# princeton-computational-imaging/Neural-Volume-Super-Resolution

Measured on AMD Instinct MI355X. Metric: rendered rays/sec (64+128 samples) at 800x800 Lego-like view, higher is better.
Workload: dtype f32 as 2 f16 limbs (3 MFMA products, f32 acc); 1 GPU; Blender-'lego'-like 800x800 view, 64 coarse + 128 fine samples, tri-plane decoder (3x800^2x48 + 32^2x48 planes, 4+4x128 MLP), 1 view per GPU per step; partition=view

## Files before the change

### neural-volume-super-resolution_amd/csrc/pair_core.h

```cpp
#pragma once
#include <type_traits>
#include <utility>

#ifndef R3_DMA_AUX
#define R3_DMA_AUX 0
#endif
#ifndef R3_ABLATE
#define R3_ABLATE 0
#endif
#include "limb_core.h"
#include "side_work.h"

#ifndef R3_GATHER_NT
#define R3_GATHER_NT 0
#endif
#ifndef R3_STAMP
#define R3_STAMP 0
#endif
#if R3_STAMP == 4
#define R3_MARK(i)
#define R3_MARKB(i)
#define R3_RESET
#define R3_MARKH(i) { __builtin_amdgcn_sched_barrier(0); const unsigned long long t_ = __builtin_amdgcn_s_memtime(); stamp[i] += (float)(t_ - tprev); tprev = t_; __builtin_amdgcn_sched_barrier(0); }
#define R3_RESETH { tprev = __builtin_amdgcn_s_memtime(); }
#elif R3_STAMP == 3
#define R3_MARKH(i)
#define R3_RESETH
#define R3_MARK(i)
#define R3_MARKB(i) { __builtin_amdgcn_sched_barrier(0); const unsigned long long t_ = __builtin_amdgcn_s_memtime(); stamp[i] += (float)(t_ - tprev); tprev = t_; __builtin_amdgcn_sched_barrier(0); }
#define R3_RESET { tprev = __builtin_amdgcn_s_memtime(); }
#elif R3_STAMP
#define R3_MARKB(i)
#define R3_RESET
#define R3_MARKH(i)
#define R3_RESETH
#define R3_MARK(i) { __builtin_amdgcn_sched_barrier(0); const unsigned long long t_ = __builtin_amdgcn_s_memtime(); stamp[i] += (float)(t_ - tprev); tprev = t_; __builtin_amdgcn_sched_barrier(0); }
#else
#define R3_MARK(i)
#define R3_MARKB(i)
#define R3_RESET
#define R3_MARKH(i)
#define R3_RESETH
#endif
#ifndef R3_RELU_PK
#define R3_RELU_PK 0
#endif
#ifndef R3_BLEND_PK
#define R3_BLEND_PK 0
#endif
#ifndef R3_NO_VIEW_HOIST
#define R3_NO_VIEW_HOIST 1
#endif

namespace nvsr {

template <int LIMBS>
struct Lds3 {
    static constexpr int SLOT = 4 * kb_words(LIMBS);
    static constexpr int SMALL = 2 * SLOT;
    static constexpr int RAYS = SMALL + SMALL_FLOATS;
    static constexpr int RAY_FLOATS = LIMBS == 2 ? 8 : 20;
    static constexpr int TAP_FLOATS = LIMBS == 2 ? 8 : 0;
    static constexpr int VTAPS = RAYS + RAYS2 * RAY_FLOATS;
    static constexpr int FAR = LIMBS == 2 ? VTAPS + RAYS2 * TAP_FLOATS : -1;
    static constexpr int RES = VTAPS + RAYS2 * TAP_FLOATS + (LIMBS == 2 ? RAYS2 : 0);
    static constexpr int RES_KB = LIMBS == 2 ? 9 : 0;
    static constexpr int PTS_WORDS = 8 * RAYS2;
    static constexpr int PTS = LIMBS == 2 ? VTAPS : RES + RES_KB * kb_words(LIMBS);
    static_assert(LIMBS != 2 || RAYS2 * TAP_FLOATS >= PTS_WORDS, "the points' region fits the taps'");
    static constexpr int TOTAL = RES + RES_KB * kb_words(LIMBS) + (LIMBS == 2 ? 0 : PTS_WORDS);
};
static_assert(Lds3<3>::TOTAL * 4 <= 160 * 1024 && Lds3<2>::TOTAL * 4 <= 160 * 1024, "LDS budget");

struct Tile3 {
    f32x16 acc[4];
    f32x16 act[4];
    float D[HALF_C], F[HALF_C];
    float V[HALF_C];
    float T, cr, cg, cb, dep, ac, zc, zn;
    float raw[4];
};

struct RawTaps4 { f32x4 r[4][HALF_C / 4]; };
constexpr int GATHER_STEPS = 12 + HALF_C;
__device__ __forceinline__ void gather4_load(int k, const GatherJob& job, int h, RawTaps4& rt) {
    const int tap = k / 3, i0 = 2 * (k % 3);
#if R3_ABLATE & 1
    rt.r[tap][i0] = f32x4{job.t.nw, job.t.ne, job.t.sw, job.t.se};
    rt.r[tap][i0 + 1] = f32x4{job.t.se, job.t.ne, job.t.sw, job.t.nw};
    return;
#endif
    const int off = tap == 0 ? job.t.o00 : tap == 1 ? job.t.o01 : tap == 2 ? job.t.o10 : job.t.o11;
    const f32x4* p = reinterpret_cast<const f32x4*>(job.plane + off + HALF_C * h);
    rt.r[tap][i0] = p[i0];
    rt.r[tap][i0 + 1] = p[i0 + 1];
}
__device__ __forceinline__ void gather4_blend(int c, const GatherJob& job, const RawTaps4& rt, float (&F)[HALF_C]) {
    const int i = c >> 2, j = c & 3;
    F[c] = fmaf(rt.r[3][i][j], job.t.se, fmaf(rt.r[2][i][j], job.t.sw, fmaf(rt.r[1][i][j], job.t.ne, rt.r[0][i][j] * job.t.nw)));
}

template <int NS, bool LOADS, bool BLENDS, bool PK = false>
__device__ __forceinline__ void gather_roll(int slot, const GatherJob& jl, float (&Fl)[HALF_C], const GatherJob& jb, float (&Fb)[HALF_C], int h,
                                            RawTaps4& rt) {
    spread<72, 0, NS>(slot, [&](int v) {
        if (LOADS && v % 3 == 0) {
            const int tap = (v / 3) / 6, piece = (v / 3) % 6;
#if R3_ABLATE & 1
            rt.r[tap][piece] = f32x4{jl.t.nw, jl.t.ne, jl.t.sw, jl.t.se};
#else
            int off = tap == 0 ? jl.t.o00 : tap == 1 ? jl.t.o01 : tap == 2 ? jl.t.o10 : jl.t.o11;
#if R3_ABLATE & 2
            off = __builtin_amdgcn_readfirstlane(off);
#endif
#if R3_ABLATE & 4
            off = off & 0xffff;
            off -= off % 48;
#endif
#if R3_GATHER_NT
            rt.r[tap][piece] = __builtin_nontemporal_load(reinterpret_cast<const f32x4*>(jl.plane + off + HALF_C * h) + piece);
#else
            rt.r[tap][piece] = reinterpret_cast<const f32x4*>(jl.plane + off + HALF_C * h)[piece];
#endif
#endif
        }
        const int w = v / 18, u = v % 18;
        if constexpr (PK) {
            if (u % 3 != 2) {
                const int c = 2 * ((u / 3) * 2 + u % 3);
                if (LOADS && w == 3) {
                    f32x2_t m = f32x2_t{rt.r[0][c >> 2][c & 3], rt.r[0][c >> 2][(c & 3) + 1]} * f32x2_t{jl.t.nw, jl.t.nw};
// ... 163 lines not shown
```

### neural-volume-super-resolution_amd/csrc/render3.hip

```cpp
#include "pair_core.h"

#include "colour_order.h"
#include "occupancy.h"
#include "nvsr_internal.h"

namespace nvsr {

template <int LZ>
__device__ __forceinline__ void render_pass3_body(const SceneDev& sc, const float* __restrict__ packed, long N, int S,
                                                  const float* __restrict__ rays, const float* __restrict__ z, int lindisp,
                                                  const float* __restrict__ noise, int white,
                                                  float* __restrict__ rgb, float* __restrict__ disp,
                                                  float* __restrict__ acc, float* __restrict__ weights,
                                                  float* __restrict__ depth, float* __restrict__ raw_out, unsigned* __restrict__ flag,
                                                  float* __restrict__ live_z = nullptr, float* __restrict__ live_w = nullptr,
                                                  int* __restrict__ live_n = nullptr, const int* __restrict__ group_slot = nullptr,
                                                  const int* __restrict__ pts = nullptr, const int* __restrict__ pt_steps = nullptr, float* views = nullptr,
                                                  const int* __restrict__ kept = nullptr, const int* __restrict__ kept_n = nullptr) {
    constexpr int LIMBS = LZ & 7;
    constexpr bool ZCOMP = (LZ & 8) != 0;
    constexpr int PHASE = (LZ >> 4) & 7;
    constexpr bool FUSED = PHASE == 0, KEPT = PHASE == 4, DENSITY = PHASE == 1 || KEPT, POINTS = PHASE == 3, COLOUR = PHASE == 2 || POINTS;
    using L = Lds3<LIMBS>;
    constexpr int NP = limb_products(LIMBS);
// ... 149 lines not shown
        n2 = norm_coord(__fadd_rn(c0[2], __fmul_rn(c1[1], zc)), sc.lo[2], sc.range[2]);
    };
    auto scale_taps = [](Taps& t) NVSR_INL {
        if constexpr (LIMBS == 2) { t.nw *= F16_X_SCALE; t.ne *= F16_X_SCALE; t.sw *= F16_X_SCALE; t.se *= F16_X_SCALE; }
    };
    auto view_job = [&](const float* rtp) NVSR_INL {
        const f32x4 c2 = reinterpret_cast<const f32x4*>(rtp)[0], c3 = reinterpret_cast<const f32x4*>(rtp)[1];
        GatherJob j;
        j.plane = sc.plane[3];
        j.t.o00 = __float_as_int(c2[0]); j.t.o01 = __float_as_int(c2[1]); j.t.o10 = __float_as_int(c2[2]); j.t.o11 = __float_as_int(c2[3]);
        j.t.nw = c3[0]; j.t.ne = c3[1]; j.t.sw = c3[2]; j.t.se = c3[3];
        scale_taps(j.t);
        return j;
    };

    __syncthreads();
    if constexpr (!DENSITY) {
#pragma unroll
        for (int k2 = 0; k2 < 2; ++k2) {
            Tile3& t = k2 ? Y : X;
            const GatherJob vj = view_job(k2 ? rtY : rtX);
#pragma unroll
            for (int k = 0; k < 12; ++k) gather4_load(k, vj, lane0 >> 5, rt);
#pragma unroll
            for (int c = 0; c < HALF_C; ++c) gather4_blend(c, vj, rt, t.V);
        }
        if constexpr (POINTS) {
#pragma unroll
            for (int k2 = 0; k2 < 2; ++k2) {
                const Tile3& t = k2 ? Y : X;
                f32x4* vp = reinterpret_cast<f32x4*>(views + ((long)blk * RAYS2 + (k2 ? ownY : ownX)) * POINT_VIEW_FLOATS + HALF_C * (lane0 >> 5));
#pragma unroll
                for (int i = 0; i < HALF_C / 4; ++i) vp[i] = f32x4{t.V[4 * i], t.V[4 * i + 1], t.V[4 * i + 2], t.V[4 * i + 3]};
            }
            __syncthreads();
            if (lane0 < 32) {
#pragma unroll
                for (int c = 0; c < 3; ++c) pt_sums[ownX * 3 + c] = pt_sums[ownY * 3 + c] = 0.0f;
                pt_ray[ownX] = (int)(rayX - pt_block); pt_ray[ownY] = (int)(rayY - pt_block);
            }
            __syncthreads();
            const int eX0 = trip > 0 ? peX[0] : POINT_NONE, eY0 = trip > 0 ? peX[32] : POINT_NONE;
            eX1 = trip > 1 ? peX[RAYS2] : POINT_NONE; eY1 = trip > 1 ? peX[RAYS2 + 32] : POINT_NONE;
            point_of(eX0, ownX, slotX, liveX, X.zc, wX);
            point_of(eY0, ownY, slotY, liveY, Y.zc, wY);
            load_view(slotX, X.V); load_view(slotY, Y.V);
        }
    } else {
#pragma unroll
        for (int k2 = 0; k2 < 2; ++k2) {
            Tile3& t = k2 ? Y : X;
            float n0, n1, n2;
            point_norm(k2 ? rcY : rcX, t.zc, n0, n1, n2);
#pragma unroll
            for (int p = 0; p < 3; ++p) {
                GatherJob pj;
                pj.plane = sc.plane[p]; pj.t = pos_taps2(sc, p, n0, n1, n2); scale_taps(pj.t);
#pragma unroll
                for (int k = 0; k < 12; ++k) gather4_load(k, pj, lane0 >> 5, rt);
#pragma unroll
                for (int c = 0; c < HALF_C; ++c) gather4_blend(c, pj, rt, t.F);
#pragma unroll
                for (int c = 0; c < HALF_C; ++c) {
                    t.D[c] = p == 0 ? t.F[c] : p == 1 ? __fadd_rn(t.D[c], t.F[c]) : div3(__fadd_rn(t.D[c], t.F[c]));
                    asm volatile("" : "+v"(t.D[c]));
                }
                __builtin_amdgcn_sched_barrier(0);
            }
        }
    }
    Limbs<LIMBS> cur, fa;
    f32x2_t nsc = {-F16_ACC_UNSCALE, -F16_ACC_UNSCALE};
    asm volatile("" : "+s"(nsc));
#if R3_STAMP
    float stamp[8] = {0, 0, 0, 0, 0, 0, 0, 0};
    unsigned long long tprev = __builtin_amdgcn_s_memtime();
#endif
    constexpr bool RESIDENT = L::RES_KB > 0 && !DENSITY;
    constexpr int KB_FIRST = DENSITY ? KB_DEN0 : RESIDENT ? KB_RGB0 + 9 : KB_RGB0;
    unsigned* const res = lds + L::RES;
    if constexpr (RESIDENT) ring3_load_resident<LIMBS, L::RES_KB>(rs, res, KB_RGB0);
    unsigned* cw = const_cast<unsigned*>(ring3_issue<LIMBS, 3>(rs, KB_FIRST));
    const int steps = COLOUR || KEPT ? trip : S;
    for (int s = 0; s < steps; ++s) {
        asm volatile("" : "+v"(rs.voff), "+v"(rs.lane));
#if R3_NO_VIEW_HOIST
        if constexpr (!POINTS) {
#pragma unroll
        for (int c = 0; c < HALF_C; ++c) asm volatile("" : "+v"(X.V[c]), "+v"(Y.V[c]));
        }
#endif
        if constexpr (POINTS) { rcX = ldsf + L::RAYS + slotX * RAY3_FLOATS; rcY = ldsf + L::RAYS + slotY * RAY3_FLOATS; }
        const int lane = rs.lane, h = lane >> 5;
        const bool last = (s + 1 == S);
        if constexpr (!COLOUR && !KEPT) {
            X.zn = depth_of(zX, rcX, last ? s : s + 1);
            Y.zn = depth_of(zY, rcY, last ? s : s + 1);
        }
        const float nzX = !COLOUR && noise ? noise[rayX * S + s] : 0.0f;
        const float nzY = !COLOUR && noise ? noise[rayY * S + s] : 0.0f;
        float xn0, xn1, xn2, yn0, yn1, yn2;
        if constexpr (!KEPT) {
            point_norm(rcX, DENSITY ? X.zn : X.zc, xn0, xn1, xn2);
            point_norm(rcY, DENSITY ? Y.zn : Y.zc, yn0, yn1, yn2);
        }
        BiasPend4 bp;
        bp.slot = bounce_slot(ldsf + L::VTAPS + rs.wave * 64 * L::TAP_FLOATS + lane * 4);
        HeadPend<3> hp3;
        HeadPend<1> hp1;
        SplitPend tp;

        auto feat = [](const float (&f)[HALF_C]) NVSR_INL { return [&f](int kb, int i) NVSR_INL { return f[8 * kb + i]; }; };
        auto hid = [](const f32x16 (&a)[4], int kb0) NVSR_INL { return [&a, kb0](int kb, int i) NVSR_INL { const int k = kb0 + kb; return a[k >> 1][8 * (k & 1) + i]; }; };
        auto split_feat = [&](const float (&f)[HALF_C]) NVSR_INL { split_all<LIMBS>([&f](int i) NVSR_INL { return f[i]; }, cur); };
        auto tail_of = [&](const f32x16 (&a)[4], int kb) NVSR_INL {
            return [&a, kb, &tp](int slice, Limbs<LIMBS>& nxt) NVSR_INL { split_slice<LIMBS>(slice, [&a, kb](int i) NVSR_INL { return a[kb >> 1][8 * (kb & 1) + i]; }, nxt, tp); };
        };
        auto none = [](int) NVSR_INL {};

        GatherJob ja, jb;
        R3_MARK(0)
        ring3_sync<(ZCOMP || COLOUR || KEPT) ? 0 : 2>();
        int eX2 = POINT_NONE, eY2 = POINT_NONE;
        if constexpr (POINTS) {
            if (s + 2 < steps) { eX2 = peX[(s + 2) * RAYS2]; eY2 = peX[(s + 2) * RAYS2 + 32]; }
            point_of(eX1, ownX, slotXn, liveXn, X.zn, wXn);
            point_of(eY1, ownY, slotYn, liveYn, Y.zn, wYn);
        } else if constexpr (COLOUR) {
            X.zn = live_depth(lzX, rcX, nX, s + 1); Y.zn = live_depth(lzY, rcY, nY, s + 1);
            wXn = live_weight(lwX, nX, s + 1); wYn = live_weight(lwY, nY, s + 1);
        } else if constexpr (KEPT) {
            X.zn = depth_of(z_row(rayX), rcX, idxXn); Y.zn = depth_of(z_row(rayY), rcY, idxYn);
            point_norm(rcX, X.zn, xn0, xn1, xn2);
            point_norm(rcY, Y.zn, yn0, yn1, yn2);
        }
        unsigned* nw = (RESIDENT || DENSITY) ? nullptr : ring3_take(rs);
        float hx[3] = {0.0f, 0.0f, 0.0f};
        if constexpr (!DENSITY) {
        const unsigned* const w_view = RESIDENT ? res : cw;
        R3_MARK(1)
        R3_RESET
#define NVSR_ROLL(TL, JL, TB, JB, LOADS, BLENDS) [&](int slot) NVSR_INL { gather_roll<NSF, LOADS, BLENDS, LIMBS == 2 && R3_BLEND_PK>(slot, JL, TL.F, JB, TB.F, h, rt); }
#define NVSR_ROLL_DMA(TL, JL, TB, JB, LOADS, BLENDS, NKB, KB0) \
        [&](int slot) NVSR_INL { gather_roll<NSF, LOADS, BLENDS, LIMBS == 2 && R3_BLEND_PK>(slot, JL, TL.F, JB, TB.F, h, rt); dma_side<LIMBS, NKB>(slot, rs, nw, KB0); }
        ja.plane = sc.plane[0]; ja.t = pos_taps2(sc, 0, xn0, xn1, xn2); scale_taps(ja.t);
        split_feat(X.V);
        if constexpr (RESIDENT) limb_block<LIMBS, 3, true, true>(w_view, lane, X.acc, cur, fa, feat(X.V), NVSR_ROLL(X, ja, Y, jb, true, false), NoTail{});
        else limb_block<LIMBS, 3, true, true>(cw, lane, X.acc, cur, fa, feat(X.V), NVSR_ROLL_DMA(X, ja, Y, jb, true, false, 3, KB_RGB0 + 3), NoTail{});
        R3_MARKB(0)
        if constexpr (POINTS) load_view(slotXn, X.V);
        jb.plane = sc.plane[0]; jb.t = pos_taps2(sc, 0, yn0, yn1, yn2); scale_taps(jb.t);
        split_feat(Y.V);
        limb_block<LIMBS, 3, true, false>(w_view, lane, Y.acc, cur, fa, feat(Y.V), NVSR_ROLL(Y, jb, X, ja, true, true), NoTail{});
        R3_MARKB(1)
        if constexpr (POINTS) load_view(slotYn, Y.V);
        const unsigned* w_p0 = res + 3 * kb_words(LIMBS);
        if constexpr (!RESIDENT) {
            cw = nw;
            ring3_sync<YOUNGER_THAN_CHUNK>();
            nw = ring3_take(rs);
            w_p0 = cw;
        }
#pragma unroll
        for (int c = 0; c < HALF_C; ++c) X.D[c] = X.F[c];
        ja.plane = sc.plane[1]; ja.t = pos_taps2(sc, 1, xn0, xn1, xn2); scale_taps(ja.t);
        split_feat(X.F);
        if constexpr (RESIDENT) limb_block<LIMBS, 3, false, true>(w_p0, lane, X.acc, cur, fa, feat(X.F), NVSR_ROLL(X, ja, Y, jb, true, true), NoTail{});
        else limb_block<LIMBS, 3, false, true>(cw, lane, X.acc, cur, fa, feat(X.F), NVSR_ROLL_DMA(X, ja, Y, jb, true, true, 3, KB_RGB0 + 6), NoTail{});
        R3_MARKB(2)
#pragma unroll
        for (int c = 0; c < HALF_C; ++c) Y.D[c] = Y.F[c];
        jb.plane = sc.plane[1]; jb.t = pos_taps2(sc, 1, yn0, yn1, yn2); scale_taps(jb.t);
        split_feat(Y.F);
        limb_block<LIMBS, 3, false, false>(w_p0, lane, Y.acc, cur, fa, feat(Y.F), NVSR_ROLL(Y, jb, X, ja, true, true), NoTail{});
        R3_MARKB(3)
        const unsigned* w_p1 = res + 6 * kb_words(LIMBS);
        if constexpr (!RESIDENT) {
            cw = nw;
            ring3_sync<YOUNGER_THAN_CHUNK>();
            nw = ring3_take(rs);
            w_p1 = cw;
        }
#pragma unroll
        for (int c = 0; c < HALF_C; ++c) X.D[c] = __fadd_rn(X.D[c], X.F[c]);
        ja.plane = sc.plane[2]; ja.t = pos_taps2(sc, 2, xn0, xn1, xn2); scale_taps(ja.t);
        split_feat(X.F);
        if constexpr (RESIDENT) limb_block<LIMBS, 3, false, true>(w_p1, lane, X.acc, cur, fa, feat(X.F), NVSR_ROLL(X, ja, Y, jb, true, true), NoTail{});
        else limb_block<LIMBS, 3, false, true>(cw, lane, X.acc, cur, fa, feat(X.F), NVSR_ROLL_DMA(X, ja, Y, jb, true, true, 3, KB_RGB0 + 9), NoTail{});
        R3_MARKB(4)
#pragma unroll
        for (int c = 0; c < HALF_C; ++c) Y.D[c] = __fadd_rn(Y.D[c], Y.F[c]);
        jb.plane = sc.plane[2]; jb.t = pos_taps2(sc, 2, yn0, yn1, yn2); scale_taps(jb.t);
        split_feat(Y.F);
        limb_block<LIMBS, 3, false, false>(w_p1, lane, Y.acc, cur, fa, feat(Y.F), NVSR_ROLL(Y, jb, X, ja, true, true), NoTail{});
        R3_MARKB(5)
        if constexpr (!RESIDENT) {
            cw = nw;
            ring3_sync<YOUNGER_THAN_CHUNK>();
        }
        nw = ring3_take(rs);
#pragma unroll
        for (int c = 0; c < HALF_C; ++c) X.D[c] = div3(__fadd_rn(X.D[c], X.F[c]));
        split_feat(X.F);
        limb_block<LIMBS, 3, false, true>(cw, lane, X.acc, cur, fa, feat(X.F), NVSR_ROLL_DMA(X, ja, Y, jb, false, true, 4, KB_RGB1), NoTail{});
        R3_MARKB(6)
// ... 4 lines not shown
                                           [&](int slot) NVSR_INL { spread<RELU_STEPS, 0, NSF>(slot, [&](int k) NVSR_INL { relu_bias_step<LIMBS>(k, small + S_BIAS + 4 * HID, h, X.acc, X.act, bp, nsc); }); },
                                           tail_of(X.act, 0));
        R3_MARKB(7)
        cw = nw;
        R3_MARK(2)
        }

        auto relu_side = [&](Tile3& t, int bias_vec) NVSR_INL {
            return [&, bias_vec](int slot) NVSR_INL { spread<RELU_STEPS, 0, NSH>(slot, [&](int k) NVSR_INL { relu_bias_step<LIMBS>(k, small + S_BIAS + bias_vec * HID, h, t.acc, t.act, bp, nsc); }); };
        };
#define NVSR_HIDDEN_LAYER_(SYNC, XA_SIDE, VPREV, VTHIS, KB_NEXT_A, NKB_A, KB_NEXT_B, NKB_B, X_B_SIDE)                                \
        R3_RESETH                                                                                                                   \
        SYNC;                                                                                                                       \
        R3_MARKH(0)                                                                                                                 \
        nw = ring3_take(rs);                                                                                                        \
        R3_MARKH(1)                                                                                                                 \
        limb_block<LIMBS, 4, true, true>(cw, lane, X.acc, cur, fa, hid(X.act, 0),                                                   \
                                         [&](int slot) NVSR_INL { (XA_SIDE)(slot); dma_side<LIMBS, NKB_A>(slot, rs, nw, KB_NEXT_A); }, tail_of(Y.act, 0)); \
        R3_MARKH(2)                                                                                                                 \
        limb_block<LIMBS, 4, true, false>(cw, lane, Y.acc, cur, fa, hid(Y.act, 0), none, tail_of(X.act, 4));                        \
        R3_MARKH(3)                                                                                                                 \
        cw = nw;                                                                                                                    \
        ring3_sync<0>();                                                                                                               \
        nw = ring3_take(rs);                                                                                                        \
        R3_MARKH(4)                                                                                                                 \
        limb_block<LIMBS, 4, false, true>(cw, lane, X.acc, cur, fa, hid(X.act, 4),                                                  \
                                          [&](int slot) NVSR_INL { dma_side<LIMBS, NKB_B>(slot, rs, nw, KB_NEXT_B); }, tail_of(Y.act, 4));   \
        R3_MARKH(5)                                                                                                                 \
        X_B_SIDE;                                                                                                                   \
        R3_MARKH(6)                                                                                                                 \
        cw = nw;

#define NVSR_HIDDEN_LAYER(VPREV, ...) NVSR_HIDDEN_LAYER_(ring3_sync<0>(), relu_side(Y, VPREV), VPREV, __VA_ARGS__)
#define NVSR_YB_PLAIN(VTHIS) (limb_block<LIMBS, 4, false, false>(cw, lane, Y.acc, cur, fa, hid(Y.act, 4), relu_side(X, VTHIS), tail_of(X.act, 0)))
        if constexpr (!DENSITY) {
        NVSR_HIDDEN_LAYER(4, 5, KB_RGB1 + 4, 4, KB_RGB1 + 8, 4, NVSR_YB_PLAIN(5))
        NVSR_HIDDEN_LAYER(5, 6, KB_RGB1 + 12, 4, KB_RGB1 + 16, 4, NVSR_YB_PLAIN(6))
        NVSR_HIDDEN_LAYER(6, 7, KB_RGB1 + 20, 4, (COLOUR ? KB_FIRST : KB_DEN0), 3,
                          (limb_block<LIMBS, 4, false, false>(cw, lane, Y.acc, cur, fa, hid(Y.act, 4),
                                                              [&](int slot) NVSR_INL {
                                                                  if constexpr (COLOUR) {
                                                                      spread<RELU_STEPS, 0, NSH / 2>(slot, [&](int k) NVSR_INL { relu_bias_step<LIMBS>(k, small + S_BIAS + 7 * HID, h, X.acc, X.act, bp, nsc); });
                                                                      spread<64, NSH / 2, NSH>(slot, [&](int k) NVSR_INL { heads_side<3>(k >> 2, k & 3, small + S_RGB_W, h, X.act, hx, hp3); });
                                                                  } else relu_side(X, 7)(slot);
                                                              },
                                                              NoTail{})))
        }

        R3_MARK(3)
        if constexpr (FUSED) {
        ring3_sync<0>();
        nw = ring3_take(rs);
        split_feat(X.D);
        limb_block<LIMBS, 3, true, true>(cw, lane, X.acc, cur, fa, feat(X.D),
                                         [&](int slot) NVSR_INL {
                                             spread<RELU_STEPS, 0, NSF>(slot, [&](int k) NVSR_INL { relu_bias_step<LIMBS>(k, small + S_BIAS + 7 * HID, h, Y.acc, Y.act, bp, nsc); });
                                             spread<64, 0, NSF>(slot, [&](int k) NVSR_INL { heads_side<3>(k >> 2, k & 3, small + S_RGB_W, h, X.act, hx, hp3); });
                                             dma_side<LIMBS, 4>(slot, rs, nw, KB_DEN1);
                                         },
                                         NoTail{});
#pragma unroll
        for (int c = 0; c < 3; ++c) X.raw[c] = (hx[c] + __shfl_xor(hx[c], 32)) + small[S_HEAD_B + 1 + c];
        float hy[3] = {0.0f, 0.0f, 0.0f};
        split_feat(Y.D);
        limb_block<LIMBS, 3, true, false>(cw, lane, Y.acc, cur, fa, feat(Y.D),
                                          [&](int slot) NVSR_INL {
                                              spread<64, 0, NSF>(slot, [&](int k) NVSR_INL { heads_side<3>(k >> 2, k & 3, small + S_RGB_W, h, Y.act, hy, hp3); });
                                              spread<RELU_STEPS, 0, NSF>(slot, [&](int k) NVSR_INL { relu_bias_step<LIMBS>(k, small + S_BIAS + 0 * HID, h, X.acc, X.act, bp, nsc); });
                                          },
                                          tail_of(X.act, 0));
#pragma unroll
        for (int c = 0; c < 3; ++c) Y.raw[c] = (hy[c] + __shfl_xor(hy[c], 32)) + small[S_HEAD_B + 1 + c];
        cw = nw;

        R3_MARK(4)
        NVSR_HIDDEN_LAYER(0, 1, KB_DEN1 + 4, 4, KB_DEN1 + 8, 4, NVSR_YB_PLAIN(1))
        NVSR_HIDDEN_LAYER(1, 2, KB_DEN1 + 12, 4, KB_DEN1 + 16, 4, NVSR_YB_PLAIN(2))
        } else if constexpr (DENSITY) {
        float (&Fg)[HALF_C] = X.F;
#define NVSR_HALF(JL, HL, JB, HB, LOADS, BLENDS, NS_) gather_half<NS_, LOADS, HL, BLENDS, HB>(slot, JL, JB, Fg, h, r2)
#define NVSR_JOB(J, P, N0, N1, N2) J.plane = sc.plane[P]; J.t = pos_taps2(sc, P, N0, N1, N2); scale_taps(J.t);
        nw = ring3_take(rs);
        NVSR_JOB(ja, 0, xn0, xn1, xn2)
        split_feat(X.D);
        limb_block<LIMBS, 3, true, true>(cw, lane, X.acc, cur, fa, feat(X.D),
                                         [&](int slot) NVSR_INL { NVSR_HALF(ja, 0, ja, 0, true, false, NSF); dma_side<LIMBS, 4>(slot, rs, nw, KB_DEN1); }, NoTail{});
        split_feat(Y.D);
        limb_block<LIMBS, 3, true, false>(cw, lane, Y.acc, cur, fa, feat(Y.D),
                                          [&](int slot) NVSR_INL {
                                              spread<RELU_STEPS, 0, NSF>(slot, [&](int k) NVSR_INL { relu_bias_step<LIMBS>(k, small + S_BIAS + 0 * HID, h, X.acc, X.act, bp, nsc); });
                                              NVSR_HALF(ja, 1, ja, 0, true, true, NSF);
                                          },
                                          tail_of(X.act, 0));
        cw = nw;
#define NVSR_DEN_LAYER(VPREV, KB_NEXT_A, KB_NEXT_B, NKB_B, PRE_XA, G_XA, PRE_YA, G_YA, PRE_XB, G_XB, PRE_YB, YB_SIDE, YB_TAIL)                      \
        ring3_sync<12>();                                                                                                           \
        nw = ring3_take(rs);                                                                                                        \
        PRE_XA                                                                                                                      \
        limb_block<LIMBS, 4, true, true>(cw, lane, X.acc, cur, fa, hid(X.act, 0),                                                   \
                                         [&](int slot) NVSR_INL { relu_side(Y, VPREV)(slot); G_XA; dma_side<LIMBS, 4>(slot, rs, nw, KB_NEXT_A); }, tail_of(Y.act, 0)); \
        PRE_YA                                                                                                                      \
        limb_block<LIMBS, 4, true, false>(cw, lane, Y.acc, cur, fa, hid(Y.act, 0), [&](int slot) NVSR_INL { G_YA; }, tail_of(X.act, 4)); \
        cw = nw;                                                                                                                    \
        ring3_sync<12>();                                                                                                           \
        nw = ring3_take(rs);                                                                                                        \
        PRE_XB                                                                                                                      \
        limb_block<LIMBS, 4, false, true>(cw, lane, X.acc, cur, fa, hid(X.act, 4),                                                  \
                                          [&](int slot) NVSR_INL { G_XB; dma_side<LIMBS, NKB_B>(slot, rs, nw, KB_NEXT_B); }, tail_of(Y.act, 4)); \
        PRE_YB                                                                                                                      \
        limb_block<LIMBS, 4, false, false>(cw, lane, Y.acc, cur, fa, hid(Y.act, 4), [&](int slot) NVSR_INL { YB_SIDE; }, YB_TAIL);     \
        cw = nw;
#define NVSR_D_SET(T) _Pragma("unroll") for (int c = 0; c < HALF_C; ++c) { T.D[c] = Fg[c]; asm volatile("" : "+v"(T.D[c])); }
#define NVSR_D_ADD(T) _Pragma("unroll") for (int c = 0; c < HALF_C; ++c) { T.D[c] = __fadd_rn(T.D[c], Fg[c]); asm volatile("" : "+v"(T.D[c])); }
#define NVSR_D_AVG(T) _Pragma("unroll") for (int c = 0; c < HALF_C; ++c) { T.D[c] = div3(__fadd_rn(T.D[c], Fg[c])); asm volatile("" : "+v"(T.D[c])); }
        NVSR_DEN_LAYER(0, KB_DEN1 + 4, KB_DEN1 + 8, 4,
                       NVSR_JOB(jb, 1, xn0, xn1, xn2), NVSR_HALF(jb, 0, ja, 1, true, true, NSH),
                       NVSR_D_SET(X), NVSR_HALF(jb, 1, jb, 0, true, true, NSH),
                       NVSR_JOB(ja, 2, xn0, xn1, xn2), NVSR_HALF(ja, 0, jb, 1, true, true, NSH),
                       NVSR_D_ADD(X), relu_side(X, 1)(slot); NVSR_HALF(ja, 1, ja, 0, true, true, NSH), tail_of(X.act, 0))
        NVSR_DEN_LAYER(1, KB_DEN1 + 12, KB_DEN1 + 16, 4,
                       NVSR_JOB(jb, 0, yn0, yn1, yn2), NVSR_HALF(jb, 0, ja, 1, true, true, NSH),
                       NVSR_D_AVG(X), NVSR_HALF(jb, 1, jb, 0, true, true, NSH),
                       NVSR_JOB(ja, 1, yn0, yn1, yn2), NVSR_HALF(ja, 0, jb, 1, true, true, NSH),
                       NVSR_D_SET(Y), relu_side(X, 2)(slot); NVSR_HALF(ja, 1, ja, 0, true, true, NSH), tail_of(X.act, 0))
        float sx[1] = {0.0f};
        auto sigma_side = [&](int slot) NVSR_INL {
            spread<RELU_STEPS, 0, NSH / 2>(slot, [&](int k) NVSR_INL { relu_bias_step<LIMBS>(k, small + S_BIAS + 3 * HID, h, X.acc, X.act, bp, nsc); });
            spread<64, NSH / 2, NSH>(slot, [&](int k) NVSR_INL { heads_side<1>(k >> 2, k & 3, small + S_ALPHA_W, h, X.act, sx, hp1); });
        };
        NVSR_DEN_LAYER(2, KB_DEN1 + 20, KB_FIRST, 3,
                       NVSR_JOB(jb, 2, yn0, yn1, yn2), NVSR_HALF(jb, 0, ja, 1, true, true, NSH),
                       NVSR_D_ADD(Y), NVSR_HALF(jb, 1, jb, 0, true, true, NSH),
                       , NVSR_HALF(jb, 1, jb, 1, false, true, NSH),
                       NVSR_D_AVG(Y), sigma_side(slot), NoTail{})
#undef NVSR_DEN_LAYER
#undef NVSR_D_SET
#undef NVSR_D_ADD
#undef NVSR_D_AVG
#undef NVSR_HALF
#undef NVSR_JOB
        X.raw[3] = (sx[0] + __shfl_xor(sx[0], 32)) + small[S_HEAD_B];
        }
        if constexpr (FUSED) {
        float sx[1] = {0.0f};
        NVSR_HIDDEN_LAYER(2, 3, KB_DEN1 + 20, 4, KB_FIRST, 3,
                          (limb_block<LIMBS, 4, false, false>(cw, lane, Y.acc, cur, fa, hid(Y.act, 4),
                                                              [&](int slot) NVSR_INL {
                                                                  spread<RELU_STEPS, 0, NSH / 2>(slot, [&](int k) NVSR_INL { relu_bias_step<LIMBS>(k, small + S_BIAS + 3 * HID, h, X.acc, X.act, bp, nsc); });
                                                                  spread<64, NSH / 2, NSH>(slot, [&](int k) NVSR_INL { heads_side<1>(k >> 2, k & 3, small + S_ALPHA_W, h, X.act, sx, hp1); });
                                                              },
                                                              NoTail{})))
        X.raw[3] = (sx[0] + __shfl_xor(sx[0], 32)) + small[S_HEAD_B];
        }
        R3_MARK(5)
        if constexpr (!COLOUR) {

        float zsX = 0.0f, zsY = 0.0f;
        int e1X = 0, e1Y = 0, e2X = 0, e2Y = 0;
        const bool lastX = KEPT ? idxX + 1 == S : last, lastY = KEPT ? idxY + 1 == S : last;
        if constexpr (KEPT) {
            zsX = depth_of(z_row(rayX), rcX, lastX ? idxX : idxX + 1); zsY = depth_of(z_row(rayY), rcY, lastY ? idxY : idxY + 1);
            { const int* kX = kept_row(rayX); e1X = kX[s + 1 < S ? s + 1 : S - 1]; e2X = kX[s + 2 < S ? s + 2 : S - 1]; }
            { const int* kY = kept_row(rayY); e1Y = kY[s + 1 < S ? s + 1 : S - 1]; e2Y = kY[s + 2 < S ? s + 2 : S - 1]; }
        }
#pragma unroll
        for (int k = 0; k < RELU_STEPS; ++k) relu_bias_step<LIMBS>(k, small + S_BIAS + 3 * HID, h, Y.acc, Y.act, bp, nsc);
        {
            float hd[1];
            head_dots<1>(small + S_ALPHA_W, h, Y.act, hd);
            Y.raw[3] = hd[0] + small[S_HEAD_B];
        }
        if (raw_out && lane < 32) {
            if (validX) *reinterpret_cast<f32x4*>(raw_out + (rayX * S + s) * 4) = f32x4{X.raw[0], X.raw[1], X.raw[2], X.raw[3]};
            if (validY) *reinterpret_cast<f32x4*>(raw_out + (rayY * S + s) * 4) = f32x4{Y.raw[0], Y.raw[1], Y.raw[2], Y.raw[3]};
        }
        if constexpr (!KEPT) actX = actY = true;
        if constexpr (KEPT) {
            {
                const float t0 = X.T, d0 = X.dep, a0 = X.ac, g0 = X.zn;
                X.zn = zsX;
                composite_weight(X, reinterpret_cast<const f32x4*>(rcX)[1][2], 0.0f, lastX);
                X.zn = g0; X.T = actX ? X.T : t0; X.dep = actX ? X.dep : d0; X.ac = actX ? X.ac : a0;
            }
            {
                const float t0 = Y.T, d0 = Y.dep, a0 = Y.ac, g0 = Y.zn;
                Y.zn = zsY;
                composite_weight(Y, reinterpret_cast<const f32x4*>(rcY)[1][2], 0.0f, lastY);
                Y.zn = g0; Y.T = actY ? Y.T : t0; Y.dep = actY ? Y.dep : d0; Y.ac = actY ? Y.ac : a0;
            }
        } else if constexpr (DENSITY) {
            composite_weight(X, reinterpret_cast<const f32x4*>(rcX)[1][2], nzX, last);
            composite_weight(Y, reinterpret_cast<const f32x4*>(rcY)[1][2], nzY, last);
        } else {
            composite_sample(X, reinterpret_cast<const f32x4*>(rcX)[1][2], nzX, last);
            composite_sample(Y, reinterpret_cast<const f32x4*>(rcY)[1][2], nzY, last);
        }
        if (weights && lane < 32) {
            if (validX && actX) weights[rayX * S + (KEPT ? idxX : s)] = X.raw[3];
            if (validY && actY) weights[rayY * S + (KEPT ? idxY : s)] = Y.raw[3];
        }
        if constexpr (DENSITY) {
            const bool liveX = actX && !(X.raw[3] == 0.0f), liveY = actY && !(Y.raw[3] == 0.0f);
            if (lane < 32) {
                if (validX && liveX) { live_z[rayX * S + cX] = ZCOMP ? __int_as_float(KEPT ? idxX : s) : X.zc; live_w[rayX * S + cX] = X.raw[3]; }
                if (validY && liveY) { live_z[rayY * S + cY] = ZCOMP ? __int_as_float(KEPT ? idxY : s) : Y.zc; live_w[rayY * S + cY] = Y.raw[3]; }
            }
            cX += liveX; cY += liveY;
            if constexpr (KEPT) {
                actX = validX && s + 1 < S && e1X >= 0; actY = validY && s + 1 < S && e1Y >= 0;
                idxX = e1X < 0 ? idxX : e1X; idxY = e1Y < 0 ? idxY : e1Y;
                idxXn = e2X < 0 ? idxX : e2X; idxYn = e2Y < 0 ? idxY : e2Y;
            }
        }
        } else {
#pragma unroll
        for (int c = 0; c < 3; ++c) X.raw[c] = (hx[c] + __shfl_xor(hx[c], 32)) + small[S_HEAD_B + 1 + c];
#pragma unroll
        for (int k = 0; k < RELU_STEPS; ++k) relu_bias_step<LIMBS>(k, small + S_BIAS + 7 * HID, h, Y.acc, Y.act, bp, nsc);
        {
            float hd[3];
            head_dots<3>(small + S_RGB_W, h, Y.act, hd);
#pragma unroll
            for (int c = 0; c < 3; ++c) Y.raw[c] = hd[c] + small[S_HEAD_B + 1 + c];
        }
        if constexpr (POINTS) {
            if (lane < 32) {
#pragma unroll
                for (int c = 0; c < 3; ++c) { pt_exch[ownX * 3 + c] = colour_term(wX, X.raw[c]); pt_exch[ownY * 3 + c] = colour_term(wY, Y.raw[c]); }
                pt_slot[ownX] = liveX ? slotX : -1; pt_slot[ownY] = liveY ? slotY : -1;
            }
            __syncthreads();
            const int p = rs.wave * 64 + lane, sl = pt_slot[p];
            if (sl >= 0 && (p == 0 || pt_slot[p - 1] != sl)) {
                float a0 = pt_sums[sl * 3], a1 = pt_sums[sl * 3 + 1], a2 = pt_sums[sl * 3 + 2];
                int q = p;
                do {
                    a0 = __fadd_rn(a0, pt_exch[q * 3]); a1 = __fadd_rn(a1, pt_exch[q * 3 + 1]); a2 = __fadd_rn(a2, pt_exch[q * 3 + 2]);
                    ++q;
                } while (q < RAYS2 && pt_slot[q] == sl);
                pt_sums[sl * 3] = a0; pt_sums[sl * 3 + 1] = a1; pt_sums[sl * 3 + 2] = a2;
            }
            __syncthreads();
            slotX = slotXn; slotY = slotYn; liveX = liveXn; liveY = liveYn; eX1 = eX2; eY1 = eY2;
        } else {
            composite_colour(X, wX, s < nX);
            composite_colour(Y, wY, s < nY);
        }
        wX = wXn; wY = wYn;
        }
#undef NVSR_HIDDEN_LAYER
#undef NVSR_HIDDEN_LAYER_
#undef NVSR_ROLL
#undef NVSR_ROLL_DMA
#undef NVSR_YB_PLAIN
        X.zc = X.zn; Y.zc = Y.zn;
        R3_MARK(6)
    }
#if R3_STAMP
    if (raw_out && rs.lane < 32 && validX) {
        for (int i = 0; i < 8; ++i) raw_out[(rayX * S + (i >> 2)) * 4 + (i & 3)] = stamp[i] / (float)S;
    }
#endif
    asm volatile("s_waitcnt vmcnt(0)" ::: "memory");

    if constexpr (POINTS) {
        if (rs.lane < 32) {
            X.cr = pt_sums[ownX * 3]; X.cg = pt_sums[ownX * 3 + 1]; X.cb = pt_sums[ownX * 3 + 2];
            Y.cr = pt_sums[ownY * 3]; Y.cg = pt_sums[ownY * 3 + 1]; Y.cb = pt_sums[ownY * 3 + 2];
        }
    }
    if (rs.lane < 32) {
#pragma unroll
        for (int k = 0; k < 2; ++k) {
            const Tile3& t = k ? Y : X;
            const long ray = k ? rayY : rayX;
            if (!(k ? validY : validX)) continue;
            float cr = t.cr, cg = t.cg, cb = t.cb;
            const float ac = COLOUR ? acc[ray] : t.ac;
            if constexpr (!COLOUR) {
                const float q = t.dep / t.ac;
                disp[ray] = 1.0f / ((q != q) ? q : fmaxf(1e-10f, q));
                acc[ray] = t.ac;
                if (depth) depth[ray] = t.dep;
            }
            if constexpr (DENSITY) {
                live_n[ray] = k ? cY : cX;
                cr = cg = cb = 0.0f;
            } else {
                if (white) { const float bg = 1.0f - ac; cr += bg; cg += bg; cb += bg; }
                rgb[ray * 3 + 0] = cr; rgb[ray * 3 + 1] = cg; rgb[ray * 3 + 2] = cb;
            }
            if (LIMBS == 2 && flag && !(fabsf(cr + cg + cb + ac) <= 3.0e38f)) __hip_atomic_fetch_or(flag, 1u, __ATOMIC_RELAXED, __HIP_MEMORY_SCOPE_AGENT);
        }
    }
}

template <int LIMBS>
__global__ __launch_bounds__(TPB2, 1) void render_pass3_coarse_kernel(SceneDev sc, const float* __restrict__ packed, long N, int S,
                                                                     const float* __restrict__ rays, const float* __restrict__ z,
                                                                     const float* __restrict__ noise, int white,
                                                                     float* __restrict__ rgb, float* __restrict__ disp,
                                                                     float* __restrict__ acc, float* __restrict__ weights,
                                                                     float* __restrict__ depth, float* __restrict__ raw_out, unsigned* __restrict__ flag) {
    render_pass3_body<LIMBS>(sc, packed, N, S, rays, z, 0, noise, white, rgb, disp, acc, weights, depth, raw_out, flag);
}
template <int LIMBS>
__global__ __launch_bounds__(TPB2, 1) void render_pass3_coarse_z_kernel(SceneDev sc, const float* __restrict__ packed, long N, int S,
                                                                       const float* __restrict__ rays, int lindisp,
                                                                       const float* __restrict__ noise, int white,
                                                                       float* __restrict__ rgb, float* __restrict__ disp,
                                                                       float* __restrict__ acc, float* __restrict__ weights,
                                                                       float* __restrict__ depth, float* __restrict__ raw_out, unsigned* __restrict__ flag) {
#if defined(__HIP_DEVICE_COMPILE__)
    render_pass3_body<LIMBS + 8>(sc, packed, N, S, rays, nullptr, lindisp, noise, white, rgb, disp, acc, weights, depth, raw_out, flag);
#endif
}
template <int LIMBS>
__global__ __launch_bounds__(TPB2, 1) void render_pass3_kernel(SceneDev sc, const float* __restrict__ packed, long N, int S,
                                                              const float* __restrict__ rays, const float* __restrict__ z,
                                                              const float* __restrict__ noise, int white,
                                                              float* __restrict__ rgb, float* __restrict__ disp,
                                                              float* __restrict__ acc, float* __restrict__ depth,
                                                              float* __restrict__ raw_out, unsigned* __restrict__ flag) {
    render_pass3_body<LIMBS>(sc, packed, N, S, rays, z, 0, noise, white, rgb, disp, acc, nullptr, depth, raw_out, flag);
}

template <int LIMBS>
__global__ __launch_bounds__(TPB2, 1) void render_pass3_density_kernel(SceneDev sc, const float* __restrict__ packed, long N, int S,
                                                                      const float* __restrict__ rays, const float* __restrict__ z,
                                                                      const float* __restrict__ noise, float* __restrict__ disp,
                                                                      float* __restrict__ acc, float* __restrict__ weights,
                                                                      float* __restrict__ depth, unsigned* __restrict__ flag,
                                                                      float* __restrict__ live_z, float* __restrict__ live_w, int* __restrict__ live_n) {
#if defined(__HIP_DEVICE_COMPILE__)
    render_pass3_body<LIMBS + 16>(sc, packed, N, S, rays, z, 0, noise, 0, nullptr, disp, acc, weights, depth, nullptr, flag, live_z, live_w, live_n);
#endif
}
template <int LIMBS>
__global__ __launch_bounds__(TPB2, 1) void render_pass3_density_z_kernel(SceneDev sc, const float* __restrict__ packed, long N, int S,
                                                                        const float* __restrict__ rays, int lindisp,
                                                                        const float* __restrict__ noise, float* __restrict__ disp,
                                                                        float* __restrict__ acc, float* __restrict__ weights,
                                                                        float* __restrict__ depth, unsigned* __restrict__ flag,
// ... 240 lines not shown
```

### neural-volume-super-resolution_amd/csrc/side_work.h

```cpp
#pragma once
#include "tile_pair.h"

namespace nvsr {

struct RawTaps2 { f32x4 r0[HALF_C / 4], r1[HALF_C / 4]; };

struct GatherJob {
    const float* plane;
    Taps t;
};

template <int G0 = 0>
__device__ __forceinline__ void gather_side(int g_, int j, const GatherJob& job, int h, RawTaps2& rt, float (&F)[HALF_C]) {
    const int g = g_ - G0;
    if ((g == 0 || g == 1 || g == 11 || g == 12) && j < 3) {
        const int off = (g == 0) ? job.t.o00 : (g == 1) ? job.t.o01 : (g == 11) ? job.t.o10 : job.t.o11;
        const f32x4* p = reinterpret_cast<const f32x4*>(job.plane + off + HALF_C * h);
#pragma unroll
        for (int i = 2 * j; i < 2 * j + 2; ++i) {
            if (g == 0 || g == 11) rt.r0[i] = p[i]; else rt.r1[i] = p[i];
        }
    }
    if (g >= 8 && g <= 10) {
#pragma unroll
        for (int k = 2 * j; k < 2 * j + 2; ++k) {
            const int c = 8 * (g - 8) + k, i = c >> 2, jj = c & 3;
            F[c] = fmaf(rt.r1[i][jj], job.t.ne, rt.r0[i][jj] * job.t.nw);
        }
    }
    if (g >= 20 && g <= 22) {
#pragma unroll
        for (int k = 2 * j; k < 2 * j + 2; ++k) {
            const int c = 8 * (g - 20) + k, i = c >> 2, jj = c & 3;
            F[c] = fmaf(rt.r1[i][jj], job.t.se, fmaf(rt.r0[i][jj], job.t.sw, F[c]));
        }
    }
}

template <int NH>
struct HeadPend { f32x4 w[NH]; };
template <int NH>
__device__ __forceinline__ void heads_side(int g, int j, const float* w, int h, const f32x16 (&in)[4], float (&s)[NH], HeadPend<NH>& pend) {
    if (g >= 0 && g < 16) {
        if (j == 0) {
#pragma unroll
            for (int n = 0; n < NH; ++n) pend.w[n] = *reinterpret_cast<const f32x4*>(w + n * HID + g * 8 + h * 4);
        }
        if (j == 2) {
#pragma unroll
            for (int e = 0; e < 4; ++e)
#pragma unroll
                for (int n = 0; n < NH; ++n) s[n] = fmaf(in[g >> 2][4 * (g & 3) + e], pend.w[n][e], s[n]);
        }
    }
}
template <class TileT>
__device__ __forceinline__ void composite_sample(TileT& t, float nrm, float noise, bool last) {
    const float dist = __fmul_rn(last ? 1e10f : __fsub_rn(t.zn, t.zc), nrm);
    const float sn = __fadd_rn(t.raw[3], noise);
    const float sig = sn < 0.0f ? 0.0f : sn;
    const float alpha = __fsub_rn(1.0f, expf(-__fmul_rn(sig, dist)));
    const float w = __fmul_rn(alpha, t.T);
    t.T = __fmul_rn(t.T, __fadd_rn(__fsub_rn(1.0f, alpha), 1e-10f));
    t.cr = __fadd_rn(t.cr, __fmul_rn(w, 1.0f / (1.0f + expf(-t.raw[0]))));
    t.cg = __fadd_rn(t.cg, __fmul_rn(w, 1.0f / (1.0f + expf(-t.raw[1]))));
    t.cb = __fadd_rn(t.cb, __fmul_rn(w, 1.0f / (1.0f + expf(-t.raw[2]))));
    t.dep = __fadd_rn(t.dep, __fmul_rn(w, t.zc));
    t.ac = __fadd_rn(t.ac, w);
    t.raw[3] = w;
}

template <class TileT>
__device__ __forceinline__ void composite_weight(TileT& t, float nrm, float noise, bool last) {
    const float dist = __fmul_rn(last ? 1e10f : __fsub_rn(t.zn, t.zc), nrm);
    const float sn = __fadd_rn(t.raw[3], noise);
    const float sig = sn < 0.0f ? 0.0f : sn;
    const float alpha = __fsub_rn(1.0f, expf(-__fmul_rn(sig, dist)));
    const float w = __fmul_rn(alpha, t.T);
    t.T = __fmul_rn(t.T, __fadd_rn(__fsub_rn(1.0f, alpha), 1e-10f));
    t.dep = __fadd_rn(t.dep, __fmul_rn(w, t.zc));
    t.ac = __fadd_rn(t.ac, w);
    t.raw[3] = w;
}
__device__ __forceinline__ float colour_term(float w, float raw) { return __fmul_rn(w, 1.0f / (1.0f + expf(-raw))); }
template <class TileT>
__device__ __forceinline__ void composite_colour(TileT& t, float w, bool live) {
    const float cr = __fadd_rn(t.cr, colour_term(w, t.raw[0]));
    const float cg = __fadd_rn(t.cg, colour_term(w, t.raw[1]));
    const float cb = __fadd_rn(t.cb, colour_term(w, t.raw[2]));
    t.cr = live ? cr : t.cr; t.cg = live ? cg : t.cg; t.cb = live ? cb : t.cb;
}

__device__ __forceinline__ Taps pos_taps2(const SceneDev& sc, int d, float n0, float n1, float n2) {
    const float* M = sc.proj + 6 * d;
    return make_taps(sc, d, n0 * M[0] + n1 * M[2] + n2 * M[4], n0 * M[1] + n1 * M[3] + n2 * M[5]);
}

}
```

Before: 8.014 million rays/s.

## Defer density compositing and Y head by one step, overlapping it with the next step's MFMA

In the density-only phase with two limbs, the Y tile's last ReLU/head work and both tiles' volume-compositing weight updates are deferred by one sample step. They are interleaved as side work inside the next step's first-layer MFMA blocks, and the per-ray state is parked in LDS tap space between steps. An epilogue finishes the final sample after the loop. The aim is to hide the serial composite tail and head reduction behind matrix work. In exchange it adds LDS traffic, register pressure and bookkeeping complexity, and it reuses the tap region, which is only safe without bounce.

```diff
diff --git a/neural-volume-super-resolution_amd/csrc/pair_core.h b/neural-volume-super-resolution_amd/csrc/pair_core.h
--- a/neural-volume-super-resolution_amd/csrc/pair_core.h
+++ b/neural-volume-super-resolution_amd/csrc/pair_core.h
@@ -47,6 +47,9 @@
 #endif
 #ifndef R3_BLEND_PK
 #define R3_BLEND_PK 0
+#endif
+#ifndef R3_DENSITY_TAIL
+#define R3_DENSITY_TAIL 1
 #endif
 #ifndef R3_NO_VIEW_HOIST
 #define R3_NO_VIEW_HOIST 1
diff --git a/neural-volume-super-resolution_amd/csrc/render3.hip b/neural-volume-super-resolution_amd/csrc/render3.hip
--- a/neural-volume-super-resolution_amd/csrc/render3.hip
+++ b/neural-volume-super-resolution_amd/csrc/render3.hip
@@ -255,6 +255,41 @@
     if constexpr (RESIDENT) ring3_load_resident<LIMBS, L::RES_KB>(rs, res, KB_RGB0);
     unsigned* cw = const_cast<unsigned*>(ring3_issue<LIMBS, 3>(rs, KB_FIRST));
     const int steps = COLOUR || KEPT ? trip : S;
+    constexpr bool ROT = R3_DENSITY_TAIL != 0 && PHASE == 1 && LIMBS == 2;
+    float pzX = 0.0f, pzY = 0.0f;
+    auto park_of = [&](int lane, int k2) NVSR_INL { return (lds_f32x4_p)(ldsf + L::VTAPS + (rs.wave * 64 + (lane & 31)) * 8 + (k2 < 2 ? 4 * k2 : 32 * 8)); };
+    auto park_store = [&](const Tile3& t, int lane, int k2) NVSR_INL { *park_of(lane, k2) = f32x4{t.zc, t.zn, t.T, t.dep}; };
+    auto park_load = [&](Tile3& t, float& pz, int lane, int k2) NVSR_INL {
+        lds_f32x4_p p = park_of(lane, k2);
+        asm volatile("" : "+v"(p));
+        const f32x4 v = *p;
+        pz = v[0]; t.zc = v[1]; t.T = v[2]; t.dep = v[3];
+    };
+    auto park_store_acc = [&](int lane) NVSR_INL { *park_of(lane, 2) = f32x4{X.ac, __int_as_float(cX), Y.ac, __int_as_float(cY)}; };
+    auto park_load_acc = [&](int lane) NVSR_INL {
+        lds_f32x4_p p = park_of(lane, 2);
+        asm volatile("" : "+v"(p));
+        const f32x4 v = *p;
+        X.ac = v[0]; cX = __float_as_int(v[1]); Y.ac = v[2]; cY = __float_as_int(v[3]);
+    };
+    if constexpr (ROT) {
+        static_assert(L::TAP_FLOATS == 8 && !R3_BOUNCE, "the parked state lives in the wave's tap region");
+#pragma unroll
+        for (int i = 0; i < 4; ++i) Y.acc[i] = f32x16{0, 0, 0, 0, 0, 0, 0, 0, 0, 0, 0, 0, 0, 0, 0, 0};
+        X.raw[3] = 0.0f;
+        X.zn = X.zc; Y.zn = Y.zc;
+        park_store(X, rs.lane, 0); park_store(Y, rs.lane, 1); park_store_acc(rs.lane);
+    }
+    auto tail_stores = [&](const Tile3& t, long ray, bool valid, bool on, int lane, int sp, float zc, int& c) NVSR_INL {
+        const bool live = on && !(t.raw[3] == 0.0f);
+        asm volatile("" : "+v"(ray));
+        const long row = ray * S;
+        if (lane < 32 && valid) {
+            if (weights && on) weights[row + sp] = t.raw[3];
+            if (live) { live_z[row + c] = ZCOMP ? __int_as_float(sp) : zc; live_w[row + c] = t.raw[3]; }
+        }
+        c += live;
+    };
     for (int s = 0; s < steps; ++s) {
         asm volatile("" : "+v"(rs.voff), "+v"(rs.lane));
 #if R3_NO_VIEW_HOIST
@@ -267,11 +302,12 @@
         const int lane = rs.lane, h = lane >> 5;
         const bool last = (s + 1 == S);
         if constexpr (!COLOUR && !KEPT) {
-            X.zn = depth_of(zX, rcX, last ? s : s + 1);
-            Y.zn = depth_of(zY, rcY, last ? s : s + 1);
-        }
-        const float nzX = !COLOUR && noise ? noise[rayX * S + s] : 0.0f;
-        const float nzY = !COLOUR && noise ? noise[rayY * S + s] : 0.0f;
+            X.zn = depth_of(ROT ? z_row(rayX) : zX, rcX, last ? s : s + 1);
+            Y.zn = depth_of(ROT ? z_row(rayY) : zY, rcY, last ? s : s + 1);
+        }
+        auto noise_at = [&](long ray, int k) NVSR_INL -> float { asm volatile("" : "+v"(ray)); return noise[ray * S + k]; };
+        const float nzX = COLOUR || !noise ? 0.0f : ROT ? noise_at(rayX, s > 0 ? s - 1 : 0) : noise[rayX * S + s];
+        const float nzY = COLOUR || !noise ? 0.0f : ROT ? noise_at(rayY, s > 0 ? s - 1 : 0) : noise[rayY * S + s];
         float xn0, xn1, xn2, yn0, yn1, yn2;
         if constexpr (!KEPT) {
             point_norm(rcX, DENSITY ? X.zn : X.zc, xn0, xn1, xn2);
@@ -294,6 +330,7 @@
         GatherJob ja, jb;
         R3_MARK(0)
         ring3_sync<(ZCOMP || COLOUR || KEPT) ? 0 : 2>();
+        if constexpr (DENSITY) { R3_MARK(1) }
         int eX2 = POINT_NONE, eY2 = POINT_NONE;
         if constexpr (POINTS) {
             if (s + 2 < steps) { eX2 = peX[(s + 2) * RAYS2]; eY2 = peX[(s + 2) * RAYS2 + 32]; }
@@ -464,17 +501,43 @@
 #define NVSR_JOB(J, P, N0, N1, N2) J.plane = sc.plane[P]; J.t = pos_taps2(sc, P, N0, N1, N2); scale_taps(J.t);
         nw = ring3_take(rs);
         NVSR_JOB(ja, 0, xn0, xn1, xn2)
+        const bool pending = s > 0;
+        WeightPend wp;
+        float sy[1] = {0.0f};
         split_feat(X.D);
         limb_block<LIMBS, 3, true, true>(cw, lane, X.acc, cur, fa, feat(X.D),
-                                         [&](int slot) NVSR_INL { NVSR_HALF(ja, 0, ja, 0, true, false, NSF); dma_side<LIMBS, 4>(slot, rs, nw, KB_DEN1); }, NoTail{});
+                                         [&](int slot) NVSR_INL {
+                                             if constexpr (ROT) {
+                                                 spread<RELU_STEPS, 0, NSF>(slot, [&](int k) NVSR_INL {
+                                                     relu_bias_step<LIMBS>(k, small + S_BIAS + 3 * HID, h, Y.acc, Y.act, bp, nsc);
+                                                     if (k == RELU_STEPS - 1) heads_side<1>(15, 2, small + S_ALPHA_W, h, Y.act, sy, hp1);
+                                                     else if (k >= 8 && (k & 3) == 0) heads_side<1>((k - 8) >> 2, 2, small + S_ALPHA_W, h, Y.act, sy, hp1);
+                                                     if (k >= 4 && k <= 64 && (k & 3) == 0) heads_side<1>((k - 4) >> 2, 0, small + S_ALPHA_W, h, Y.act, sy, hp1);
+                                                 });
+                                                 if (slot == 0) { park_load(X, pzX, lane, 0); park_load_acc(lane); }
+                                                 spread<5, 0, NSF / 3>(slot, [&](int k) NVSR_INL { composite_weight_step(k, X, pzX, X.zc, rcX, nzX, false, pending, wp); });
+                                                 if (slot == NSF / 3 + 1) { tail_stores(X, rayX, validX, pending, lane, s - 1, pzX, cX); park_store(X, lane, 0); }
+                                             }
+                                             NVSR_HALF(ja, 0, ja, 0, true, false, NSF); dma_side<LIMBS, 4>(slot, rs, nw, KB_DEN1);
+                                         }, NoTail{});
         split_feat(Y.D);
         limb_block<LIMBS, 3, true, false>(cw, lane, Y.acc, cur, fa, feat(Y.D),
                                           [&](int slot) NVSR_INL {
                                               spread<RELU_STEPS, 0, NSF>(slot, [&](int k) NVSR_INL { relu_bias_step<LIMBS>(k, small + S_BIAS + 0 * HID, h, X.acc, X.act, bp, nsc); });
+                                              if constexpr (ROT) {
+                                                  if (slot == 0) {
+                                                      park_load(Y, pzY, lane, 1);
+                                                      const auto sw = __builtin_amdgcn_permlane32_swap(__float_as_uint(sy[0]), __float_as_uint(sy[0]), false, false);
+                                                      Y.raw[3] = (sy[0] + __uint_as_float(h ? sw[0] : sw[1])) + small[S_HEAD_B];
+                                                  }
+                                                  spread<5, 1, NSF / 3>(slot, [&](int k) NVSR_INL { composite_weight_step(k, Y, pzY, Y.zc, rcY, nzY, false, pending, wp); });
+                                                  if (slot == NSF / 3 + 1) { tail_stores(Y, rayY, validY, pending, lane, s - 1, pzY, cY); park_store(Y, lane, 1); park_store_acc(lane); }
+                                              }
                                               NVSR_HALF(ja, 1, ja, 0, true, true, NSF);
                                           },
                                           tail_of(X.act, 0));
         cw = nw;
+        R3_MARK(4)
 #define NVSR_DEN_LAYER(VPREV, KB_NEXT_A, KB_NEXT_B, NKB_B, PRE_XA, G_XA, PRE_YA, G_YA, PRE_XB, G_XB, PRE_YB, YB_SIDE, YB_TAIL)                      \
         ring3_sync<12>();                                                                                                           \
         nw = ring3_take(rs);                                                                                                        \
@@ -521,6 +584,10 @@
 #undef NVSR_D_AVG
 #undef NVSR_HALF
 #undef NVSR_JOB
+        if constexpr (ROT) {
+            const auto sw = __builtin_amdgcn_permlane32_swap(__float_as_uint(sx[0]), __float_as_uint(sx[0]), false, false);
+            X.raw[3] = (sx[0] + __uint_as_float(h ? sw[0] : sw[1])) + small[S_HEAD_B];
+        } else
         X.raw[3] = (sx[0] + __shfl_xor(sx[0], 32)) + small[S_HEAD_B];
         }
         if constexpr (FUSED) {
@@ -535,7 +602,8 @@
         X.raw[3] = (sx[0] + __shfl_xor(sx[0], 32)) + small[S_HEAD_B];
         }
         R3_MARK(5)
-        if constexpr (!COLOUR) {
+        if constexpr (ROT) {
+        } else if constexpr (!COLOUR) {
 
         float zsX = 0.0f, zsY = 0.0f;
         int e1X = 0, e1Y = 0, e2X = 0, e2Y = 0;
@@ -635,12 +703,38 @@
 #undef NVSR_ROLL
 #undef NVSR_ROLL_DMA
 #undef NVSR_YB_PLAIN
-        X.zc = X.zn; Y.zc = Y.zn;
+        if constexpr (!ROT) { X.zc = X.zn; Y.zc = Y.zn; }
         R3_MARK(6)
+    }
+    if constexpr (ROT) {
+        park_load(X, pzX, rs.lane, 0); park_load(Y, pzY, rs.lane, 1); park_load_acc(rs.lane);
+        if (S > 0) {
+            const int lane = rs.lane, h = lane >> 5;
+            BiasPend4 bp;
+            bp.slot = bounce_slot(ldsf + L::VTAPS + rs.wave * 64 * L::TAP_FLOATS + lane * 4);
+#pragma unroll
+            for (int k = 0; k < RELU_STEPS; ++k) relu_bias_step<LIMBS>(k, small + S_BIAS + 3 * HID, h, Y.acc, Y.act, bp, nsc);
+            float hd[1];
+            head_dots<1>(small + S_ALPHA_W, h, Y.act, hd);
+            Y.raw[3] = hd[0] + small[S_HEAD_B];
+            const float nzX = noise ? noise[rayX * S + S - 1] : 0.0f, nzY = noise ? noise[rayY * S + S - 1] : 0.0f;
+            WeightPend wp;
+#pragma unroll
+            for (int k = 0; k < 5; ++k) composite_weight_step(k, X, pzX, pzX, rcX, nzX, true, true, wp);
+#pragma unroll
+            for (int k = 0; k < 5; ++k) composite_weight_step(k, Y, pzY, pzY, rcY, nzY, true, true, wp);
+            tail_stores(X, rayX, validX, true, lane, S - 1, pzX, cX);
+            tail_stores(Y, rayY, validY, true, lane, S - 1, pzY, cY);
+        }
     }
 #if R3_STAMP
     if (raw_out && rs.lane < 32 && validX) {
         for (int i = 0; i < 8; ++i) raw_out[(rayX * S + (i >> 2)) * 4 + (i & 3)] = stamp[i] / (float)S;
+    }
+    if constexpr (DENSITY) {
+        if (weights && S >= 8 && rs.lane < 32 && validX) {
+            for (int i = 0; i < 8; ++i) weights[rayX * S + i] = stamp[i] / (float)S;
+        }
     }
 #endif
     asm volatile("s_waitcnt vmcnt(0)" ::: "memory");
diff --git a/neural-volume-super-resolution_amd/csrc/side_work.h b/neural-volume-super-resolution_amd/csrc/side_work.h
--- a/neural-volume-super-resolution_amd/csrc/side_work.h
+++ b/neural-volume-super-resolution_amd/csrc/side_work.h
@@ -82,6 +82,20 @@
     t.ac = __fadd_rn(t.ac, w);
     t.raw[3] = w;
 }
+struct WeightPend { float dist, sn, e, alpha, w; };
+template <class TileT>
+__device__ __forceinline__ void composite_weight_step(int k, TileT& t, float zc, float zn, const float* rc, float noise, bool last, bool on, WeightPend& p) {
+    if (k == 0) { p.dist = __fmul_rn(last ? 1e10f : __fsub_rn(zn, zc), rc[6]); p.sn = __fadd_rn(t.raw[3], noise); }
+    if (k == 1) { const float sig = p.sn < 0.0f ? 0.0f : p.sn; p.e = -__fmul_rn(sig, p.dist); }
+    if (k == 2) p.e = expf(p.e);
+    if (k == 3) { p.alpha = __fsub_rn(1.0f, p.e); p.w = __fmul_rn(p.alpha, t.T); }
+    if (k == 4) {
+        const float T = __fmul_rn(t.T, __fadd_rn(__fsub_rn(1.0f, p.alpha), 1e-10f));
+        const float dep = __fadd_rn(t.dep, __fmul_rn(p.w, zc)), ac = __fadd_rn(t.ac, p.w);
+        t.T = on ? T : t.T; t.dep = on ? dep : t.dep; t.ac = on ? ac : t.ac;
+        t.raw[3] = p.w;
+    }
+}
 __device__ __forceinline__ float colour_term(float w, float raw) { return __fmul_rn(w, 1.0f / (1.0f + expf(-raw))); }
 template <class TileT>
 __device__ __forceinline__ void composite_colour(TileT& t, float w, bool live) {
```

Result: no change. 8.086 million rays/s (median of 6 runs) (+0.9%).
